# feiyeha/EGM-Unet

Measured on AMD Instinct MI355X. Metric: train images/sec at 3x512x512 bs=8/GPU, higher is better.
Workload: dtype bf16; 1 GPU; EGM-UNet GRFBUNet(3,2,base_c=32) fwd+5-term-loss+bwd+SGD, 8x3x512x512 per GPU (BASELINE.json configs[1]); global_batch=8, parallelism=dp1, launch=hipGraph replay, world_size=1

## Files before the change

### egm_unet_amd/csrc/conv_wgrad.hip

```cpp
#include "common.h"
#include "group.h"
#include <string.h>
#include <stdio.h>
#include <stdlib.h>
#include <type_traits>

typedef __attribute__((ext_vector_type(8))) __bf16 bf16x8_t;
typedef __attribute__((ext_vector_type(4))) short s16x4_t;
typedef __attribute__((ext_vector_type(8))) short s16x8_t;
typedef __attribute__((ext_vector_type(16))) float f32x16_t;
typedef __attribute__((ext_vector_type(4))) unsigned int u32x4_t;

int egm_conv_c7_wgrad_plan(int dtype, int N, int H, int W, int Cin, int Cout, int KH, int KW, int dil);
int egm_conv_c7_wgrad_launch(const void* x, int ldx, const void* dy, int lddy, float* slab, int nslab, int N, int H, int W, egm_stream_t s);
int egm_conv_c16d_wgrad_plan(int dtype, int N, int H, int W, int Cin, int Cout, int KH, int KW, int dil);
int egm_conv_c16d_wgrad_launch(const void* x, int ldx, const void* dy, int lddy, float* slab, int nslab, int N, int H, int W, int dil,
                               egm_stream_t s);

namespace {

constexpr int TH = 8, TW = 32;
constexpr int kMaxRowDil = 36;

template <typename T> struct WMma;
// ... 674 lines not shown
    if (sl == 0 && i < total) {
        s = (red[e] + red[64 + e]) + (red[128 + e] + red[192 + e]);
        const int ci = (int)(i % CinP), co = (int)((i / CinP) % CoutP), tap = (int)(i / ((long long)CinP * CoutP));
        if (co < CoutR && ci < CinR && (co / cout_g) == (ci / cin_g)) {
            const long long o = ((long long)co * cin_g + (ci % cin_g)) * taps + tap;
            dw[o] = accumulate ? dw[o] + s : s;
        }
    }
}


__global__ __launch_bounds__(1024) void wgrad_reduce_wide_kernel(const float* __restrict__ slab, float* __restrict__ dw, int nslab, int taps,
                                                                 int CoutP, int CinP, int CoutR, int CinR, int groups, int accumulate) {
    __shared__ float red[1024];
    const long long total = (long long)taps * CoutP * CinP;
    const int cin_g = CinR / groups, cout_g = CoutR / groups;
    const int e = threadIdx.x & 63, sl = threadIdx.x >> 6;
    const long long i = (long long)blockIdx.x * 64 + e;
    float s = 0.f;
    if (i < total)
        for (int k = sl; k < nslab; k += 16) s += slab[(long long)k * total + i];
    red[threadIdx.x] = s;
    __syncthreads();
    for (int w = 8; w > 0; w >>= 1) {
        if (sl < w) red[threadIdx.x] += red[threadIdx.x + w * 64];
        __syncthreads();
    }
    if (sl == 0 && i < total) {
        s = red[e];
        const int ci = (int)(i % CinP), co = (int)((i / CinP) % CoutP), tap = (int)(i / ((long long)CinP * CoutP));
        if (co < CoutR && ci < CinR && (co / cout_g) == (ci / cin_g)) {
            const long long o = ((long long)co * cin_g + (ci % cin_g)) * taps + tap;
            dw[o] = accumulate ? dw[o] + s : s;
        }
    }
}

struct WredEntry { const float* slab; float* dw; int nslab, taps, CoutP, CinP, CoutR, CinR, groups, accumulate, chunk0, pad; };
constexpr int kWredElems = 256;
__global__ __launch_bounds__(256) void wgrad_reduce_multi_kernel(const WredEntry* __restrict__ tab, int n) {
    __shared__ float4 red[256];
    const int s_t = egm_find_entry(tab, n, (long long)blockIdx.x);
    const int s_c = (int)((long long)blockIdx.x - (long long)tab[s_t].chunk0);
    const WredEntry w = tab[s_t];
    const long long total = (long long)w.taps * w.CoutP * w.CinP;
    const int cin_g = w.CinR / w.groups, cout_g = w.CoutR / w.groups;
    const int e = threadIdx.x & 63, sl = threadIdx.x >> 6;
    const long long i0 = (long long)s_c * kWredElems + e * 4;
    float4 s = make_float4(0.f, 0.f, 0.f, 0.f);
    if (i0 < total) {
        const float* src = w.slab + i0;
        int k = sl;
        for (; k + 4 < w.nslab; k += 8) {
            const float4 a = *reinterpret_cast<const float4*>(src + (long long)k * total);
            const float4 c = *reinterpret_cast<const float4*>(src + (long long)(k + 4) * total);
            s.x += a.x; s.y += a.y; s.z += a.z; s.w += a.w;
            s.x += c.x; s.y += c.y; s.z += c.z; s.w += c.w;
        }
        if (k < w.nslab) {
            const float4 a = *reinterpret_cast<const float4*>(src + (long long)k * total);
            s.x += a.x; s.y += a.y; s.z += a.z; s.w += a.w;
        }
    }
    red[threadIdx.x] = s;
    __syncthreads();
    if (sl == 0 && i0 < total) {
        const float4 r0 = red[e], r1 = red[64 + e], r2 = red[128 + e], r3 = red[192 + e];
        const float v[4] = {(r0.x + r1.x) + (r2.x + r3.x), (r0.y + r1.y) + (r2.y + r3.y), (r0.z + r1.z) + (r2.z + r3.z),
                            (r0.w + r1.w) + (r2.w + r3.w)};
#pragma unroll
        for (int j = 0; j < 4; ++j) {
            const long long i = i0 + j;
            const int ci = (int)(i % w.CinP), co = (int)((i / w.CinP) % w.CoutP), tap = (int)(i / ((long long)w.CinP * w.CoutP));
            if (co < w.CoutR && ci < w.CinR && (co / cout_g) == (ci / cin_g)) {
                const long long o = ((long long)co * cin_g + (ci % cin_g)) * w.taps + tap;
                w.dw[o] = w.accumulate ? w.dw[o] + v[j] : v[j];
            }
        }
    }
}

struct WgradPlan { int A, B, C, ntaps, ngroups, nsplit, nco_tiles, nci_tiles, npt, tiles_y, tiles_x, dma, ws, c7; size_t smem; long long slab_bytes; };

int wgrad_plan(int dtype, int N, int H, int W, int Cin, int Cout, int KH, int KW, int dil, WgradPlan* pl) {
    if (KH == 1 && KW == 1) dil = 1;
    pl->c7 = 0;
    {
        const int ns = egm_conv_c7_wgrad_plan(dtype, N, H, W, Cin, Cout, KH, KW, dil);
        if (ns > 0) {
            memset(pl, 0, sizeof(*pl));
            pl->c7 = 1; pl->ntaps = 7; pl->ngroups = 7; pl->nsplit = ns; pl->A = pl->B = 1; pl->C = 4;
            pl->slab_bytes = (long long)ns * KH * KW * Cout * Cin * (long long)sizeof(float);
            return EGM_OK;
        }
        const int nd = egm_conv_c16d_wgrad_plan(dtype, N, H, W, Cin, Cout, KH, KW, dil);
        if (nd > 0) {
            memset(pl, 0, sizeof(*pl));
            pl->c7 = 2; pl->ntaps = 3; pl->ngroups = 3; pl->nsplit = nd; pl->A = pl->B = 1; pl->C = 4;
            pl->slab_bytes = (long long)nd * KH * KW * Cout * Cin * (long long)sizeof(float);
            return EGM_OK;
        }
    }
    if (dil == 1) {
        if (KH == 3 && KW == 3) { pl->ntaps = 9; pl->ngroups = 1; }
        else if (KH == 1 && KW == 1) { pl->ntaps = 1; pl->ngroups = 1; }
        else if (KW == 5) { pl->ntaps = 5; pl->ngroups = KH; }
        else if (KW == 7) { pl->ntaps = 7; pl->ngroups = KH; }
        else return EGM_ERR_UNSUPPORTED;
    } else {
        const int rbp = dtype == EGM_BF16 ? 64 : 128;
        const int Ap = (dtype == EGM_F32 && Cout > 32 && Cin > 32) ? 1 : (Cout > 32 ? 2 : 1), Bp = Cin > 32 ? 2 : 1;
        const size_t row_smem = (size_t)Ap * TH * TW * rbp + (size_t)Bp * TH * (TW + 2 * dil) * rbp;
        if (KH == 3 && KW == 3 && dil <= kMaxRowDil && row_smem <= 156 * 1024 && W >= 128 && H >= 128 && Cin <= 32 && Cout <= 32) { pl->ntaps = 3; pl->ngroups = 3; }
        else { pl->ntaps = 1; pl->ngroups = KH * KW; }
    }
    int A = Cout > 32 ? 2 : 1, B = Cin > 32 ? 2 : 1;
    if (dtype == EGM_F32 && A * B == 4) A = 1;
    pl->A = A; pl->B = B; pl->C = 4 / (A * B);
    pl->nco_tiles = egm_cdiv(Cout, 32 * A); pl->nci_tiles = egm_cdiv(Cin, 32 * B);
    pl->tiles_y = egm_cdiv(H, TH); pl->tiles_x = egm_cdiv(W, TW); pl->npt = N * pl->tiles_y * pl->tiles_x;
    const int blocks_per_split = pl->nco_tiles * pl->nci_tiles * pl->ngroups;
    static const int per_cu_small = getenv("EGM_WGRAD_PER_CU") ? atoi(getenv("EGM_WGRAD_PER_CU")) : 2;
    static const int ws_on = getenv("EGM_WGRAD_WS") ? atoi(getenv("EGM_WGRAD_WS")) : 1;
    const bool ws_family = dtype == EGM_BF16 && ws_on && pl->ntaps >= 5;
    pl->ws = ws_family ? 1 : 0;
    int per_cu = ws_family ? 1 : ((pl->ntaps <= 3 && dtype == EGM_BF16) ? per_cu_small : 1);
    static const int ws_per_cu = getenv("EGM_WGRAD_WS_PER_CU") ? atoi(getenv("EGM_WGRAD_WS_PER_CU")) : 1;
    if (ws_family && ws_per_cu > 1 && A * B == 1 && pl->ntaps == 9) per_cu = ws_per_cu;
    int nsplit = 256 * per_cu / blocks_per_split;
    if (nsplit < 1) nsplit = 1;
    if (nsplit > pl->npt) nsplit = pl->npt;
    pl->nsplit = nsplit;
    const int rb = dtype == EGM_BF16 ? 64 : 128;
    const int wh = pl->ntaps == 9 ? 3 : 1, ww = pl->ntaps == 9 ? 3 : pl->ntaps;
    const int pw = (dil > 1 && pl->ntaps == 3) ? TW + 2 * dil : TW + ww - 1;
    pl->smem = (size_t)A * TH * TW * rb + (size_t)B * (TH + wh - 1) * pw * rb;
    static const int dma_off = getenv("EGM_WGRAD_NO_DMA") != nullptr;
    pl->dma = (dtype == EGM_BF16 && !pl->ws && !dma_off && A * B == 4 && pl->ntaps == 9 && 2 * pl->smem <= 156 * 1024) ? 1 : 0;
    if (pl->ws) pl->smem = (size_t)A * TH * TW * rb + (((size_t)B * (TH + wh - 1) * pw * rb + 4095) & ~(size_t)4095);
    if (pl->dma || pl->ws) pl->smem *= 2;
    const size_t red_bytes = pl->C > 1 ? (size_t)A * B * (pl->C - 1) * pl->ntaps * 16 * 64 * sizeof(float) : 0;
    if (pl->smem < red_bytes) pl->smem = red_bytes;
    pl->slab_bytes = (long long)nsplit * KH * KW * Cout * Cin * (long long)sizeof(float);
    return EGM_OK;
}

template <typename Single, typename Multi>
int launch_wgrad_group_impl(const EgmGroupRec* recs, int n, hipStream_t st, Single single, Multi multi, int threads, const char* what) {
    if (n == 1) {
        WgradParams first;
        memcpy(&first, recs[0].params, sizeof(WgradParams));
        const int* g3 = reinterpret_cast<const int*>(recs[0].params + sizeof(WgradParams));
        hipLaunchKernelGGL(single, dim3(g3[0], g3[1], g3[2]), dim3(threads), recs[0].smem, st, first);
        EGM_CHECK_LAUNCH(what);
        return EGM_OK;
    }
    WgradMulti m;
    size_t smem = 0;
    m.n = n; m.blk0[0] = 0;
    for (int i = 0; i < n; ++i) {
        memcpy(&m.p[i], recs[i].params, sizeof(WgradParams));
        const int* g3 = reinterpret_cast<const int*>(recs[i].params + sizeof(WgradParams));
        m.nx[i] = g3[0]; m.ny[i] = g3[1];
        m.blk0[i + 1] = m.blk0[i] + g3[0] * g3[1] * g3[2];
        if (recs[i].smem > smem) smem = recs[i].smem;
    }
    for (int i = n; i < EGM_GROUP_MAX; ++i) { m.p[i] = m.p[0]; m.nx[i] = m.ny[i] = 1; m.blk0[i + 1] = m.blk0[n]; }
    hipLaunchKernelGGL(multi, dim3(m.blk0[n]), dim3(threads), smem, st, m);
    EGM_CHECK_LAUNCH(what);
    return EGM_OK;
}
template <typename T, int NTAPS>
int launch_wgrad_group(const EgmGroupRec* recs, int n, hipStream_t st) {
    static bool attr_done = false;
    if (!attr_done) {
        hipError_t e = hipFuncSetAttribute(reinterpret_cast<const void*>(conv_wgrad_multi_kernel<T, NTAPS>),
                                           hipFuncAttributeMaxDynamicSharedMemorySize, 160 * 1024);
        if (e != hipSuccess) EGM_FAIL(EGM_ERR_LAUNCH, "conv_wgrad_multi: hipFuncSetAttribute: %s", hipGetErrorString(e));
        attr_done = true;
    }
    return launch_wgrad_group_impl(recs, n, st, conv_wgrad_kernel<T, NTAPS>, conv_wgrad_multi_kernel<T, NTAPS>, 256, "conv_wgrad (group)");
}
template <int NTAPS, int CC>
int launch_wgrad_ws_group(const EgmGroupRec* recs, int n, hipStream_t st) {
    static bool attr_done = false;
    if (!attr_done) {
        hipError_t e = hipFuncSetAttribute(reinterpret_cast<const void*>(conv_wgrad_ws_multi_kernel<NTAPS, CC>),
                                           hipFuncAttributeMaxDynamicSharedMemorySize, 160 * 1024);
        if (e != hipSuccess) EGM_FAIL(EGM_ERR_LAUNCH, "conv_wgrad_ws_multi: hipFuncSetAttribute: %s", hipGetErrorString(e));
        attr_done = true;
    }
    return launch_wgrad_group_impl(recs, n, st, conv_wgrad_ws_kernel<NTAPS, CC>, conv_wgrad_ws_multi_kernel<NTAPS, CC>, 512, "conv_wgrad_ws (group)");
}
inline bool wgrad_record(int (*fn)(const EgmGroupRec*, int, hipStream_t), const WgradParams& p, dim3 grid, size_t smem) {
    if (!egm_group_recording()) return false;
    static_assert(sizeof(WgradParams) + 3 * sizeof(int) <= sizeof(EgmGroupRec::params), "group record too small");
    EgmGroupRec r;
    r.launch = fn;
    memcpy(r.params, &p, sizeof(WgradParams));
    const int g3[3] = {(int)grid.x, (int)grid.y, (int)grid.z};
    memcpy(r.params + sizeof(WgradParams), g3, sizeof(g3));
    r.G = 0; r.grid = (int)(grid.x * grid.y * grid.z); r.smem = smem;
    egm_group_push(r);
    return true;
}
template <typename T, int NTAPS>
int launch_wgrad_4w(const WgradParams& p, const WgradPlan& pl, hipStream_t st) {
    static bool attr_done = false;
    if (!attr_done) {
        hipError_t e = hipFuncSetAttribute(reinterpret_cast<const void*>(conv_wgrad_kernel<T, NTAPS>),
                                           hipFuncAttributeMaxDynamicSharedMemorySize, 160 * 1024);
        if (e != hipSuccess) EGM_FAIL(EGM_ERR_LAUNCH, "conv_wgrad: hipFuncSetAttribute: %s", hipGetErrorString(e));
        attr_done = true;
    }
// ... 5 lines not shown
}
template <int NTAPS, int CC>
int launch_wgrad_ws_rot(const WgradParams& p, const WgradPlan& pl, hipStream_t st) {
    static bool attr_done = false;
    if (!attr_done) {
        hipError_t e = hipFuncSetAttribute(reinterpret_cast<const void*>(conv_wgrad_ws_kernel<NTAPS, CC>),
                                           hipFuncAttributeMaxDynamicSharedMemorySize, 160 * 1024);
        if (e != hipSuccess) EGM_FAIL(EGM_ERR_LAUNCH, "conv_wgrad_ws: hipFuncSetAttribute: %s", hipGetErrorString(e));
        attr_done = true;
    }
    dim3 grid(pl.nsplit, pl.nco_tiles * pl.nci_tiles, pl.ngroups);
    if (wgrad_record(&launch_wgrad_ws_group<NTAPS, CC>, p, grid, pl.smem)) return EGM_OK;
    hipLaunchKernelGGL((conv_wgrad_ws_kernel<NTAPS, CC>), grid, dim3(512), pl.smem, st, p);
    EGM_CHECK_LAUNCH("conv_wgrad_ws");
    return EGM_OK;
}
template <int NTAPS>
int launch_wgrad_ws(const WgradParams& p, const WgradPlan& pl, hipStream_t st) {
    if constexpr (NTAPS == 9) {
        static const bool rot_on = getenv("EGM_WGRAD_ROT") ? atoi(getenv("EGM_WGRAD_ROT")) != 0 : true;
        if (rot_on) {
            if (pl.C == 1) return launch_wgrad_ws_rot<NTAPS, 1>(p, pl, st);
            if (pl.C == 2) return launch_wgrad_ws_rot<NTAPS, 2>(p, pl, st);
            return launch_wgrad_ws_rot<NTAPS, 4>(p, pl, st);
        }
    }
    return launch_wgrad_ws_rot<NTAPS, 0>(p, pl, st);
}
template <typename T, int NTAPS>
int launch_wgrad(const WgradParams& p, const WgradPlan& pl, hipStream_t st) {
    if constexpr (sizeof(T) == 2 && NTAPS >= 5) {
        if (pl.ws) return launch_wgrad_ws<NTAPS>(p, pl, st);
    }
    return launch_wgrad_4w<T, NTAPS>(p, pl, st);
}

template <typename T>
int dispatch_wgrad(const WgradParams& p, const WgradPlan& pl, hipStream_t st) {
    switch (pl.ntaps) {
        case 9: return launch_wgrad<T, 9>(p, pl, st);
        case 7: return launch_wgrad<T, 7>(p, pl, st);
        case 5: return launch_wgrad<T, 5>(p, pl, st);
        case 3: return launch_wgrad<T, 3>(p, pl, st);
        case 1: return launch_wgrad<T, 1>(p, pl, st);
    }
    EGM_FAIL(EGM_ERR_UNSUPPORTED, "conv_wgrad: unsupported tap group %d", pl.ntaps);
}

}

extern "C" long long egm_conv_wgrad_workspace(int N, int H, int W, int Cin, int Cout, int KH, int KW) {
    WgradPlan pl;
    if (wgrad_plan(EGM_F32, N, H, W, Cin, Cout, KH, KW, 1, &pl) != EGM_OK) return -1;
    long long a = pl.slab_bytes;
    if (wgrad_plan(EGM_BF16, N, H, W, Cin, Cout, KH, KW, 1, &pl) != EGM_OK) return -1;
    if (pl.slab_bytes > a) a = pl.slab_bytes;
    if (wgrad_plan(EGM_BF16, N, H, W, Cin, Cout, KH, KW, 2, &pl) != EGM_OK) return -1;
    if (pl.slab_bytes > a) a = pl.slab_bytes;
    if (wgrad_plan(EGM_F32, N, H, W, Cin, Cout, KH, KW, 2, &pl) != EGM_OK) return -1;
    if (pl.slab_bytes > a) a = pl.slab_bytes;
    return a;
}

extern "C" int egm_conv_wgrad_kernel_name(int dtype, int N, int H, int W, int Cin, int Cout, int KH, int KW, int dil, char* buf, int buflen) {
    WgradPlan pl;
    if (KH == 1 && KW == 1) dil = 1;
    if (wgrad_plan(dtype, N, H, W, Cin, Cout, KH, KW, dil, &pl) != EGM_OK) return -1;
    char tmp[96];
    static const bool rot_on = getenv("EGM_WGRAD_ROT") ? atoi(getenv("EGM_WGRAD_ROT")) != 0 : true;
    if (pl.c7) snprintf(tmp, sizeof(tmp), pl.c7 == 1 ? "conv7x7_c16_wgrad_kernel" : "conv3x3d_c16_wgrad_kernel");
    else if (dtype == EGM_BF16 && pl.ws)
        snprintf(tmp, sizeof(tmp), "conv_wgrad_ws_kernel<%d, %d>", pl.ntaps, (pl.ntaps == 9 && rot_on) ? pl.C : 0);
    else
        snprintf(tmp, sizeof(tmp), "conv_wgrad_kernel<%s, %d>", dtype == EGM_BF16 ? "bf16_t" : "float", pl.ntaps);
    const int n = (int)strlen(tmp);
    if (buf != nullptr && buflen > 0) { strncpy(buf, tmp, (size_t)buflen - 1); buf[buflen - 1] = 0; }
    return n;
}
extern "C" int egm_conv_wgrad_slabs(int dtype, int N, int H, int W, int Cin, int Cout, int KH, int KW, int dil) {
    WgradPlan pl;
    if (KH == 1 && KW == 1) dil = 1;
    if (wgrad_plan(dtype, N, H, W, Cin, Cout, KH, KW, dil, &pl) != EGM_OK) return -1;
    return pl.nsplit;
}
extern "C" int egm_wgrad_reduce_chunk(void) { return kWredElems; }
extern "C" int egm_wgrad_reduce_multi(const void* table_dev, int n, long long total_chunks, egm_stream_t s) {
    EGM_REQUIRE(table_dev && n > 0 && total_chunks > 0 && total_chunks < (1LL << 30), "wgrad_reduce_multi: bad args");
    hipLaunchKernelGGL(wgrad_reduce_multi_kernel, dim3((unsigned)total_chunks), dim3(256), 0, (hipStream_t)s, (const WredEntry*)table_dev, n);
    EGM_CHECK_LAUNCH("wgrad_reduce_multi");
    return EGM_OK;
}

extern "C" int egm_conv_wgrad(int dtype, const void* x, int ldx, const void* dy, int lddy, float* dw, void* workspace, int N,
                              int H, int W, int Cin, int Cout, int CinR, int CoutR, int KH, int KW, int dil, int groups,
                              int accumulate, egm_stream_t s) {
    EGM_REQUIRE(x && dy && workspace, "conv_wgrad: null pointer");
    EGM_REQUIRE(N > 0 && H > 0 && W > 0, "conv_wgrad: bad shape");
    EGM_REQUIRE(Cin % 8 == 0 && Cout % 8 == 0 && Cin > 0 && Cout > 0, "conv_wgrad: padded channels must be multiples of 8");
    EGM_REQUIRE(CinR <= Cin && CoutR <= Cout && CinR > 0 && CoutR > 0 && groups > 0 && CinR % groups == 0 && CoutR % groups == 0,
                "conv_wgrad: bad real channel counts");
    EGM_REQUIRE(ldx >= Cin && lddy >= Cout && ldx % 8 == 0 && lddy % 8 == 0, "conv_wgrad: bad ld");
    EGM_REQUIRE(egm_aligned16(x) && egm_aligned16(dy) && egm_aligned16(workspace), "conv_wgrad: pointers must be 16-byte aligned");
    EGM_REQUIRE(dil >= 1 && (KH & 1) && (KW & 1), "conv_wgrad: bad kernel");
    if (KH == 1 && KW == 1) dil = 1;
    WgradPlan pl;
    if (wgrad_plan(dtype, N, H, W, Cin, Cout, KH, KW, dil, &pl) != EGM_OK)
        EGM_FAIL(EGM_ERR_UNSUPPORTED, "conv_wgrad: unsupported kernel %dx%d dil %d", KH, KW, dil);
    EGM_REQUIRE(pl.smem <= 160 * 1024, "conv_wgrad: LDS budget exceeded");
    WgradParams p;
    p.x = x; p.dy = dy; p.slab = (float*)workspace; p.ldx = ldx; p.lddy = lddy; p.N = N; p.H = H; p.W = W;
    p.Cin = Cin; p.Cout = Cout; p.KH = KH; p.KW = KW; p.dil = dil; p.tiles_y = pl.tiles_y; p.tiles_x = pl.tiles_x;
    p.npt = pl.npt; p.nsplit = pl.nsplit; p.A = pl.A; p.B = pl.B; p.C = pl.C; p.nci_tiles = pl.nci_tiles; p.ngroups = pl.ngroups;
    p.dma = pl.dma;
    hipStream_t st = (hipStream_t)s;
    int rc;
    const bool paused = dw != nullptr && egm_group_recording();
    if (paused) egm_group_set_recording(false);
    if (pl.c7 == 1) rc = egm_conv_c7_wgrad_launch(x, ldx, dy, lddy, (float*)workspace, pl.nsplit, N, H, W, s);
    else if (pl.c7 == 2) rc = egm_conv_c16d_wgrad_launch(x, ldx, dy, lddy, (float*)workspace, pl.nsplit, N, H, W, dil, s);
    else if (dtype == EGM_BF16) rc = dispatch_wgrad<bf16_t>(p, pl, st);
    else if (dtype == EGM_F32) rc = dispatch_wgrad<float>(p, pl, st);
    else rc = EGM_ERR_ARG;
    if (paused) egm_group_set_recording(true);
    if (rc == EGM_ERR_ARG && dtype != EGM_BF16 && dtype != EGM_F32) EGM_FAIL(EGM_ERR_ARG, "conv_wgrad: unknown dtype %d", dtype);
    if (rc != EGM_OK) return rc;
    if (dw == nullptr) return EGM_OK;
    return egm_wgrad_reduce((const float*)workspace, dw, pl.nsplit, KH * KW, Cout, Cin, CoutR, CinR, groups, accumulate, s);
}

extern "C" int egm_conv_wgrad_multi(int dtype, const egm_conv_wgrad_desc* d, int n, egm_stream_t s) {
    EGM_REQUIRE(d && n > 0 && n <= EGM_WGRAD_MULTI_MAX, "conv_wgrad_multi: 1..%d convolutions per call", EGM_WGRAD_MULTI_MAX);
    EGM_REQUIRE(!egm_group_recording(), "conv_wgrad_multi: called inside an open launch group");
    int rc = egm_group_begin();
    if (rc != EGM_OK) return rc;
    for (int i = 0; i < n && rc == EGM_OK; ++i)
        rc = egm_conv_wgrad(dtype, d[i].x, d[i].ldx, d[i].dy, d[i].lddy, nullptr, d[i].slabs, d[i].N, d[i].H, d[i].W, d[i].Cin, d[i].Cout, d[i].Cin_real,
                            d[i].Cout_real, d[i].KH, d[i].KW, d[i].dil, d[i].groups, 0, s);
    if (rc != EGM_OK) { egm_group_abort(); return rc; }
    return egm_group_end(s);
}

extern "C" int egm_wgrad_reduce(const float* slabs, float* dw, int nslab, int taps, int CoutP, int CinP, int CoutR, int CinR, int groups,
                                int accumulate, egm_stream_t s) {
    EGM_REQUIRE(slabs && dw && nslab > 0 && taps > 0 && CoutP > 0 && CinP > 0 && CoutR > 0 && CoutR <= CoutP && CinR > 0 && CinR <= CinP && groups > 0,
                "wgrad_reduce: bad args");
    hipStream_t st = (hipStream_t)s;
    const long long total = (long long)taps * CoutP * CinP;
    const int grid = (int)((total + 63) / 64);
    if (nslab >= 256 && grid < 1024)
        hipLaunchKernelGGL(wgrad_reduce_wide_kernel, dim3(grid), dim3(1024), 0, st, slabs, dw, nslab, taps, CoutP, CinP, CoutR, CinR, groups, accumulate);
    else
        hipLaunchKernelGGL(wgrad_reduce_kernel, dim3(grid), dim3(256), 0, st, slabs, dw, nslab, taps, CoutP, CinP, CoutR, CinR, groups, accumulate);
    EGM_CHECK_LAUNCH("wgrad_reduce");
    return EGM_OK;
}
```

### egm_unet_amd/ops.py

```python
import ctypes
import os
import struct
import threading
import weakref
from collections import namedtuple

import torch
from torch.autograd import Function, Variable

from ._lib import ACT_NONE, ACT_RELU, ACT_SIGMOID, dtype_code, lib, ptr, stream


def pad8(c: int) -> int:
    return (c + 7) // 8 * 8


def _nhwc(t: torch.Tensor):
    assert t.dim() == 4, t.shape
    N, H, W, C = t.shape
    s = t.stride()
    ok = (s[3] == 1 and s[2] % 8 == 0 and s[2] >= C and s[1] == W * s[2] and s[0] == H * W * s[2]
          and t.data_ptr() % 16 == 0 and C % 8 == 0)
    if not ok:
        if C % 8:
            raise RuntimeError(f"egm_unet_amd: channel count {C} is not a multiple of 8")
        t = t.contiguous()
        s = t.stride()
    return t, s[2]


def _npix(t):
    return t.shape[0] * t.shape[1] * t.shape[2]


def _f32(n, device, zero=False):
    return (torch.zeros if zero else torch.empty)(n, dtype=torch.float32, device=device)


class _Switch:

    def __init__(self, env, default, doc=None, parse=lambda v: v != "0"):
        self.on, self.__doc__ = parse(os.environ.get(env, default)), doc

    def __call__(self, enabled=None):
        if enabled is not None:
            self.on = type(self.on)(enabled)
        return type(self.on)(self.on)


_zero_pools = {}


def _zero_grad_vec(n, device):
    pool = _zero_pools.get(device)
    if pool is None or pool[0].numel() < pool[1] + n:
        if torch.cuda.is_current_stream_capturing():
            return torch.zeros(n, dtype=torch.float32, device=device)
        pool = _zero_pools[device] = [torch.zeros(max(1 << 16, 4 * n), dtype=torch.float32, device=device), 0]
    off = pool[1]
    pool[1] = off + n
    return pool[0][off:off + n]


def _bn_conv_bias_grad(Cout, dy, training, device):
    return _zero_grad_vec(Cout, device) if training else _channel_sum(dy)[0, :Cout]


def _slot_or_new(out_slot, shape, dtype, device):
    if out_slot is None:
        t = torch.empty(shape, dtype=dtype, device=device)
        return t, shape[3]
    t = out_slot[0]
    v, ld = _nhwc(t)
    if v.data_ptr() != t.data_ptr() or tuple(t.shape) != tuple(shape) or t.dtype != dtype:
        raise RuntimeError(f"egm_unet_amd: output slot {tuple(t.shape)}/{t.dtype} does not fit result {tuple(shape)}/{dtype}")
    return t, ld


def cat_slots(N, H, W, channels, dtype, device):
    buf = torch.empty((N, H, W, sum(channels)), dtype=dtype, device=device)
    views, off = [], 0
    for c in channels:
        views.append(buf[..., off:off + c])
# ... 164 lines not shown
        st = model._egm_prepack = {"dtype": dtype, "convs": convs, "bufs": bufs, "table": DeviceTable(), "stamp": None}
    convs, bufs = st["convs"], st["bufs"]
    if not convs:
        return
    stamp = (_weight_generation[0], tuple(m.weight._version for m in convs), tuple(m.weight.data_ptr() for m in convs))
    if stamp == st["stamp"]:
        return
    L = lib()
    chunk = L.cdll.egm_conv_pack_chunk()
    blob, chunks = bytearray(), 0
    for m, (wf, wd) in zip(convs, bufs):
        Cout, Cin_g, KH, KW = m.weight.shape
        Cin = Cin_g * m.groups
        blob += struct.pack("<QQQiiiiiiii", m.weight.data_ptr(), wf.data_ptr(), wd.data_ptr(), Cout, Cin, pad8(Cout), pad8(Cin), KH, KW,
                            m.groups, chunks)
        chunks += (KH * KW * pad8(Cout) * pad8(Cin) + chunk - 1) // chunk
    dev = convs[0].weight.device
    table = st["table"].get(bytes(blob), dev)
    L.call("egm_conv_pack_multi", dtype_code(dtype), ptr(table), len(convs), chunks, stream())
    for m, (wf, wd) in zip(convs, bufs):
        w = m.weight
        key = (w.data_ptr(), w._version, _weight_generation[0], dtype, m.groups, tuple(w.shape))
        _pack_cache[id(w)] = (key, wf, wd, weakref.ref(w))
    st["stamp"] = stamp


_conv_uses = {}


def _note_conv_use(weight):
    ent = _conv_uses.get(id(weight))
    if ent is None or ent[0]() is not weight or ent[1] != _weight_generation[0]:
        ent = _conv_uses[id(weight)] = [weakref.ref(weight), _weight_generation[0], 0, 0]
        if len(_conv_uses) > 4096:
            for k in [k for k, v in _conv_uses.items() if v[0]() is None]:
                del _conv_uses[k]
    ent[2] += 1
    ent[3] = max(ent[3], ent[2])


def _sole_conv_use(weight):
    ent = _conv_uses.get(id(weight))
    if ent is None or ent[0]() is not weight:
        return False
    sole = ent[3] == 1
    ent[2] -= 1
    if ent[2] <= 0:
        del _conv_uses[id(weight)]
    return sole


_DEFER_WGRAD = os.environ.get("EGM_DEFER_WGRAD", "1") != "0"
merge_wgrads = _Switch("EGM_MERGE_WGRAD", "1",
                       """Get / set whether the slab kernels of deferred weight gradients are launched together when backward ends (merged
                       launches).""")
defer_bgrads = _Switch("EGM_DEFER_BGRAD", "1",
                       """Get / set whether conv bias gradients are left to the one multi-tensor pass at the end of backward.""")
fuse_dz = _Switch("EGM_FUSE_DZ", "1",
                  """Get / set whether BatchNorm backward computes dz on the fly from the classifier / MCALayer behind it (tests compare both
                  ways).""")


def _wgrad_deferrable(weight):
    return (_DEFER_WGRAD and _sole_conv_use(weight) and weight.is_leaf and weight.grad is None
            and not weight._backward_hooks and not torch.is_grad_enabled())


_wgrad_table, _wgrad_table_partial, _bgrad_table, _bgrad_table_partial = DeviceTable(), DeviceTable(), DeviceTable(), DeviceTable()
_BSUM_ENTRY = struct.Struct("<3Qq6i")
_WGRAD_DESC = struct.Struct("<3Q14i")
_wgrad_names = {}


def _wgrad_kernel_of(dt, N, H, W, CinP, CoutP, KH, KW, dil):
    key = (dt, N, H, W, CinP, CoutP, KH, KW, dil)
    name = _wgrad_names.get(key)
    if name is None:
        buf = ctypes.create_string_buffer(96)
        lib().cdll.egm_conv_wgrad_kernel_name(dt, N, H, W, CinP, CoutP, KH, KW, dil, ctypes.cast(buf, ctypes.c_void_p), 96)
        name = _wgrad_names[key] = buf.value
    return name


_Slab = namedtuple("_Slab", "dt x ldx gy ldg ws N H W CinP CoutP Cin Cout KH KW dil groups")
_Wgrad = namedtuple("_Wgrad", "ws param nslab taps CoutP CinP Cout Cin groups gref gptr")
_Bgrad = namedtuple("_Bgrad", "gy ldg npix C Cout param gref gptr")


def _handed_over(queue, ready_only, name):
    todo, later = [], []
    for ent in queue:
        grad = ent.param.grad
        if ent.gref() is not None or (grad is not None and grad.data_ptr() == ent.gptr):
            todo.append(ent)
        elif ready_only:
            later.append(ent)
        elif grad is not None:
            raise RuntimeError(f"deferred conv {name} gradient lost its destination: {name}.grad exists but is not the buffer backward() "
                               f"returned (tensor hook / gradient copy); set EGM_DEFER_{name[0].upper()}GRAD=0 for this model")
    queue[:] = later
    return todo


_runs = {}


class _BackwardRun:
    __slots__ = ("id", "slabs", "wgrads", "bgrads", "dz", "__weakref__")

    def __init__(self, run_id):
        self.id, self.slabs, self.wgrads, self.bgrads, self.dz = run_id, [], [], [], {}

    def finish(self):
        _runs.pop(self.id, None)
        if self.dz:
            kinds = [v[1][0] for v in self.dz.values()]
            self.dz.clear()
            raise RuntimeError(f"egm_unet_amd: deferred BatchNorm gradients {kinds} were never consumed (the tensor between the producer and "
                               "its BatchNorm had another consumer); call ops.fuse_dz(False)")
        self.flush()

    def flush(self, ready_only=False):
        self.flush_bgrads(ready_only)
        self.launch_slabs()
        self.reduce_wgrads(ready_only)

    def flush_bgrads(self, ready_only=False):
        todo = _handed_over(self.bgrads, ready_only, "bias") if self.bgrads else None
        if not todo:
            return
        L = lib()
        by_dtype = {}
        for e in todo:
            by_dtype.setdefault(e.gy.dtype, []).append(e)
        for dtype, ents in by_dtype.items():
            dev = ents[0].gy.device
            nblks = [L.query("egm_channel_partials_blocks", e.npix, e.C) for e in ents]
            ws = torch.empty(sum(nb * 2 * e.C for nb, e in zip(nblks, ents)), dtype=torch.float32, device=dev)
            blob1, blob2, b1, b2, off = bytearray(), bytearray(), 0, 0, 0
            for nb, e in zip(nblks, ents):
                part = ws.data_ptr() + 4 * off
                blob1 += _BSUM_ENTRY.pack(e.gy.data_ptr(), part, e.gptr, e.npix, e.ldg, e.C, e.Cout, nb, b1, 0)
                blob2 += _BSUM_ENTRY.pack(e.gy.data_ptr(), part, e.gptr, e.npix, e.ldg, e.C, e.Cout, nb, b2, 0)
                b1 += nb; b2 += e.C // 8; off += nb * 2 * e.C
            _bgrad_table.reserve(dev); _bgrad_table_partial.reserve(dev)
            table = (_bgrad_table_partial if ready_only else _bgrad_table).get(bytes(blob1 + blob2), dev)
            L.call("egm_bias_grad_multi", dtype_code(dtype), ptr(table), len(ents), b1, b2, stream())

    def launch_slabs(self):
        if not self.slabs:
            return
        L, st = lib(), stream()
        todo, self.slabs = self.slabs, []
        buckets = {}
        for e in todo:
            buckets.setdefault((e.dt, _wgrad_kernel_of(e.dt, e.N, e.H, e.W, e.CinP, e.CoutP, e.KH, e.KW, e.dil)), []).append(e)
        per = 4
        for (dt, _name), ents in buckets.items():
            for i in range(0, len(ents), per):
                blob = b"".join(_WGRAD_DESC.pack(e.x.data_ptr(), e.gy.data_ptr(), e.ws.data_ptr(), e.ldx, e.ldg, e.N, e.H, e.W, e.CinP, e.CoutP,
                                                 e.Cin, e.Cout, e.KH, e.KW, e.dil, e.groups, 0) for e in ents[i:i + per])
                L.call("egm_conv_wgrad_multi", dt, blob, len(ents[i:i + per]), st)

    def reduce_wgrads(self, ready_only=False):
        todo = _handed_over(self.wgrads, ready_only, "weight") if self.wgrads else None
        if not todo:
            return
        blob, chunks = bytearray(), 0
        per = lib().cdll.egm_wgrad_reduce_chunk()
        for e in todo:
            blob += struct.pack("<QQiiiiiiiiii", e.ws.data_ptr(), e.gptr, e.nslab, e.taps, e.CoutP, e.CinP, e.Cout, e.Cin, e.groups, 0, chunks, 0)
            chunks += (e.taps * e.CoutP * e.CinP + per - 1) // per
        dev = todo[0].param.device
        _wgrad_table.reserve(dev); _wgrad_table_partial.reserve(dev)
        table = (_wgrad_table_partial if ready_only else _wgrad_table).get(bytes(blob), dev)
        lib().call("egm_wgrad_reduce_multi", ptr(table), len(todo), chunks, stream())


def _run(create=True):
    run_id = torch._C._current_graph_task_id()
    ref = _runs.get(run_id)
    run = None if ref is None else ref()
    if run is None and create:
        run = _BackwardRun(run_id)
        _runs[run_id] = weakref.ref(run, lambda _ref: _runs.pop(run_id, None))
        Variable._execution_engine.queue_callback(run.finish)
    return run


def flush_ready_wgrads():
    run = _run(create=False)
    if run is not None:
        run.flush(ready_only=True)


def _queue_wgrad(ws, weight, nslab, taps, CoutP, CinP, Cout, Cin, groups, gw):
    _run().wgrads.append(_Wgrad(ws, weight, nslab, taps, CoutP, CinP, Cout, Cin, groups, weakref.ref(gw), gw.data_ptr()))


def _defer_dz(standin, payload):
    _run().dz[standin.data_ptr()] = (standin, payload)


def _take_dz(g):
    run = _run(create=False)
    return run.dz.pop(g.data_ptr(), None) if run is not None and run.dz else None


def _bias_grad(gy, Cout, bias=None, defer=False):
    if (defer and defer_bgrads.on and bias is not None and bias.is_leaf and bias.grad is None and not bias._backward_hooks
            and not torch.is_grad_enabled()):
        gy, ldg = _nhwc(gy)
        gb = torch.empty(Cout, dtype=torch.float32, device=gy.device)
        _run().bgrads.append(_Bgrad(gy, ldg, _npix(gy), gy.shape[3], Cout, bias, weakref.ref(gb), gb.data_ptr()))
        return gb
    return _channel_sum(gy)[0, :Cout]


def _channel_sum(t):
    t, ld = _nhwc(t)
    C, npix = t.shape[3], _npix(t)
    nb = lib().query("egm_channel_partials_blocks", npix, C)
    part = _f32(nb * 2 * C, t.device)
    out = _f32((2, C), t.device)
    lib().call("egm_channel_sums", dtype_code(t.dtype), ptr(t), ld, npix, C, ptr(part), stream())
    lib().call("egm_reduce_tiles", ptr(part), nb, C, ptr(out), stream())
    return out


class Lazy:
    __slots__ = ("y", "coef", "act")

    def __init__(self, y, coef, act):
        self.y, self.coef, self.act = y, coef, act

    shape = property(lambda self: self.y.shape)
    dtype = property(lambda self: self.y.dtype)
    device = property(lambda self: self.y.device)

    def materialize(self, out=None):
        return _Materialize.apply(self.y, self.coef, self.act, None if out is None else [out])


def materialize(x, out=None):
    if isinstance(x, Lazy):
# ... 1951 lines not shown
```

### include/egm_hip.h

```cpp
#ifndef EGM_HIP_H
#define EGM_HIP_H

#ifdef __cplusplus
extern "C" {
#endif

typedef void* egm_stream_t;

enum egm_status { EGM_OK = 0, EGM_ERR_ARG = -1, EGM_ERR_LAUNCH = -2, EGM_ERR_UNSUPPORTED = -3 };
enum egm_dtype { EGM_F32 = 0, EGM_BF16 = 1 };
enum egm_act { EGM_ACT_NONE = 0, EGM_ACT_RELU = 1, EGM_ACT_SIGMOID = 2, EGM_ACT_SILU = 3  };

int egm_version(void);
const char* egm_last_error(void);
int egm_device_ok(void);

int egm_nchw_to_nhwc(int dtype, const void* src_f32, void* dst, int ld, int N, int C, int H, int W, egm_stream_t s);
int egm_nhwc_to_nchw(int dtype, const void* src, int ld, void* dst_f32, int N, int C, int H, int W, egm_stream_t s);

int egm_conv_pack(int dtype, const void* w_oihw_f32, void* wf, void* wd, int Cout, int Cin, int KH, int KW, int groups,
                  egm_stream_t s);
int egm_conv_pack_chunk(void);
int egm_conv_pack_multi(int dtype, const void* table_dev, int n, long long total_chunks, egm_stream_t s);
int egm_group_begin(void);
int egm_group_end(egm_stream_t s);
int egm_group_abort(void);
int egm_conv_tile_mode(int mode);
int egm_conv_tile_debug(int dbg);
int egm_conv_c7_mode(int mode);
int egm_conv_split_ok(int dtype, int N, int H, int W, int Cin, int Cout, int KH, int KW, int dil, int csplit);
int egm_conv_fwd_split(int dtype, const void* x, int ldx, const void* wf, void* y, int ldy, void* y2, int ldy2, int csplit, int N,
                       int H, int W, int Cin, int Cout, int KH, int KW, int dil, egm_stream_t s);
int egm_conv_kernel_name(int dtype, int N, int H, int W, int Cin, int Cout, int KH, int KW, int dil, char* buf, int buflen);
int egm_conv_fwd(int dtype, const void* x, int ldx, const void* wf, const void* bias_f32, int bias_n, void* y, int ldy,
                 float* stats, int N, int H, int W, int Cin, int Cout, int KH, int KW, int dil, egm_stream_t s);
int egm_conv_stats_tiles(int dtype, int N, int H, int W, int Cin, int Cout, int KH, int KW, int dil);
int egm_conv_fwd_act(int dtype, const void* x, int ldx, const void* wf, const void* bias_f32, int bias_n, void* y, int ldy, int N, int H,
                     int W, int Cin, int Cout, int KH, int KW, int dil, int act, egm_stream_t s);
int egm_conv_fold_chunk(void);
int egm_conv_fold_pack_multi(int dtype, const void* table_dev, int n, long long total_chunks, egm_stream_t s);
int egm_argmax_u8(const float* logits, const unsigned char* lut, unsigned char* out, int N, int C, int H, int W, egm_stream_t s);
long long egm_conv_wgrad_workspace(int N, int H, int W, int Cin, int Cout, int KH, int KW);
int egm_conv_wgrad(int dtype, const void* x, int ldx, const void* dy, int lddy, float* dw_oihw_f32, void* workspace,
                   int N, int H, int W, int Cin, int Cout, int CinR, int CoutR, int KH, int KW, int dil, int groups,
                   int accumulate, egm_stream_t s);
int egm_conv_wgrad_kernel_name(int dtype, int N, int H, int W, int Cin, int Cout, int KH, int KW, int dil, char* buf, int buflen);
#define EGM_WGRAD_MULTI_MAX 4
typedef struct egm_conv_wgrad_desc {
    const void* x; const void* dy; void* slabs;
    int ldx, lddy, N, H, W, Cin, Cout, Cin_real, Cout_real, KH, KW, dil, groups, pad_;
} egm_conv_wgrad_desc;
int egm_conv_wgrad_multi(int dtype, const egm_conv_wgrad_desc* descs, int n, egm_stream_t stream);
int egm_conv_wgrad_slabs(int dtype, int N, int H, int W, int Cin, int Cout, int KH, int KW, int dil);
int egm_wgrad_reduce(const float* slabs, float* dw_oihw_f32, int nslab, int taps, int CoutP, int CinP, int CoutR, int CinR, int groups,
                     int accumulate, egm_stream_t s);
int egm_wgrad_reduce_chunk(void);
int egm_wgrad_reduce_multi(const void* table_dev, int n, long long total_chunks, egm_stream_t s);
int egm_dwconv3_fwd(int dtype, const void* x, int ldx, const float* w, const float* b, const float* scale, void* y, int ldy,
                    int N, int H, int W, int C, egm_stream_t s);
long long egm_dwconv3_bwd_workspace(int N, int H, int W, int C);
int egm_dwconv3_bwd(int dtype, const void* x, int ldx, const void* dy, int lddy, const float* w, const float* b,
                    const float* scale, void* dx, int lddx, float* dw, float* db, float* dscale, void* workspace,
                    int N, int H, int W, int C, egm_stream_t s);

int egm_channel_partials_blocks(long long npix, int C);
int egm_channel_sums(int dtype, const void* x, int ld, long long npix, int C, float* partials, egm_stream_t s);
int egm_reduce_tiles(const float* tiles, int ntiles, int C, float* out_2xC, egm_stream_t s);
int egm_reduce_tiles_batched(const float* tiles, int batch, int ntiles, int C, float* out, egm_stream_t s);
typedef struct { const void* x; float* part; float* out; long long npix; int ld, C, Cout, nblk, chunk0, pad; } egm_bsum_entry;
int egm_bias_grad_multi(int dtype, const void* table_dev, int n, long long blocks1, long long blocks2, egm_stream_t s);

int egm_bn_finalize(const float* stats, int ntiles, long long count, const float* gamma, const float* beta, float eps,
                    float momentum, float* running_mean, float* running_var, float* scale, float* shift,
                    float* save_mean, float* save_rstd, int C, int C_real, egm_stream_t s);
int egm_bn_eval_coeffs(const float* gamma, const float* beta, const float* running_mean, const float* running_var,
                       float eps, float* scale, float* shift, float* save_mean, float* save_rstd, int C, int C_real,
                       egm_stream_t s);
int egm_bn_act_fwd(int dtype, const void* y, int ldy, const float* scale, const float* shift, int act, void* z, int ldz,
                   long long npix, int C, egm_stream_t s);
int egm_bn_act_bwd_reduce(int dtype, const void* dz, int lddz, const void* y, int ldy, const float* scale,
                          const float* shift, const float* save_mean, const float* save_rstd, int act, float* partials,
                          long long npix, int C, egm_stream_t s);
int egm_bn_act_bwd_apply(int dtype, const void* dz, int lddz, const void* y, int ldy, const float* scale,
                         const float* shift, const float* save_mean, const float* save_rstd, int act, int train,
                         const float* sums, void* dy, int lddy, long long npix, int C, egm_stream_t s);
int egm_bn_act_cls_fwd(int dtype, const void* y, int ldy, const float* scale, const float* shift, int act, void* z, int ldz,
                       const float* w_cls, int nc, int ldw, const float* bias, float* logits_nchw, int N, int H, int W, int C,
                       egm_stream_t s);
int egm_bn_cls_bwd_reduce(int dtype, const void* dlogits, int lddl, const float* w_cls, int nc, int ldw, const void* y, int ldy,
                          const float* scale, const float* shift, const float* save_mean, const float* save_rstd, int act,
                          float* partials, long long npix, int C, egm_stream_t s);
int egm_bn_cls_bwd_apply(int dtype, const void* dlogits, int lddl, const float* w_cls, int nc, int ldw, const void* y, int ldy,
                         const float* scale, const float* shift, const float* save_mean, const float* save_rstd, int act, int train,
                         const float* sums, void* dy, int lddy, long long npix, int C, egm_stream_t s);
int egm_bn_mca_bwd_reduce(int dtype, const void* dxo, int ldd, const float* gates, const float* coef, int no_spatial, const void* y,
                          int ldy, const float* scale, const float* shift, const float* save_mean, const float* save_rstd, int act,
                          float* partials, int N, int H, int W, int C, egm_stream_t s);
int egm_bn_mca_bwd_apply(int dtype, const void* dxo, int ldd, const float* gates, const float* coef, int no_spatial, const void* y,
                         int ldy, const float* scale, const float* shift, const float* save_mean, const float* save_rstd, int act,
                         int train, const float* sums, void* dy, int lddy, int N, int H, int W, int C, egm_stream_t s);
int egm_bn_bwd_coefs(const float* partials, int ntiles, long long count, const float* scale, const float* shift,
                     const float* save_mean, const float* save_rstd, int train, float* sums_2xC, float* cf_4xC, int C,
                     egm_stream_t s);

#define EGM_BN_MULTI_MAX 4
enum egm_bn_multi_pass { EGM_BN_MULTI_FINALIZE = 0, EGM_BN_MULTI_FWD = 1, EGM_BN_MULTI_BWD_REDUCE = 2, EGM_BN_MULTI_BWD_COEFS = 3,
                         EGM_BN_MULTI_BWD_APPLY = 4 };
typedef struct egm_bn_desc {
    const void* y;  void* z;  const void* dz;  void* dy;
    float* coef;
    const float* stats;
    const float* gamma;  const float* beta;  float* running_mean;  float* running_var;
    float* partials;  float* sums;  float* cf4;
    long long npix;
    int ldy, ldz, lddz, lddy, ntiles, nblocks, C, C_real, act, train;
    float eps, momentum;
} egm_bn_desc;
int egm_bn_multi(int dtype, int pass, const egm_bn_desc* descs, int n, egm_stream_t s);

enum egm_ew_mode { EGM_EW_GATE = 0, EGM_EW_SAR = 1 };
int egm_bn_ew_fwd(int dtype, int mode, const void* y, int ldy, const float* scale, const float* shift, int act, const void* p,
                  int ldp, float alpha, void* out, int ldo, long long npix, int C, egm_stream_t s);
int egm_bn_ew_bwd_reduce(int dtype, int mode, const void* g, int ldg, const void* q, int ldq, const void* y, int ldy,
                         const float* scale, const float* shift, const float* save_mean, const float* save_rstd, int act,
                         float alpha, float* partials, long long npix, int C, egm_stream_t s);
int egm_bn_ew_bwd_apply(int dtype, int mode, const void* g, int ldg, const void* q, int ldq, const void* y, int ldy,
                        const float* cf_4xC, int act, float alpha, void* dy, int lddy, void* dp, int lddp, long long npix, int C,
                        egm_stream_t s);

typedef struct egm_pw_head {
    const void* x;  const void* w;  const void* wd;
    const float* bias;  const float* gamma;  const float* beta;  float* running_mean;  float* running_var;
    float* coef;
    const void* p;  void* out;
    const void* g;  const void* q;  void* dp;
    float* sums;  float* cf4;  float* dw;  float* dbias;
// ... 276 lines not shown
```

Baseline: 673.1 images/s.

## Cap wgrad split-K slabs for large 3x3 convs and balance multi-launch grouping

For large ws-family 3x3 weight-gradient convs with a 2x2 tile config, large slab footprint and many pixel tiles, the split count is capped so each block walks at least a minimum number of tiles. This shrinks the fp32 slab traffic and the reduction cost. On the Python side, wgrad descriptors within a kernel bucket are regrouped by a small exhaustive search. It estimates per-CU wave steps from block counts and walk lengths so the multi-launches are better balanced. The risk is lower parallelism per launch and search overhead, though results are cached and replayed under a graph.

```diff
diff --git a/egm_unet_amd/csrc/conv_wgrad.hip b/egm_unet_amd/csrc/conv_wgrad.hip
--- a/egm_unet_amd/csrc/conv_wgrad.hip
+++ b/egm_unet_amd/csrc/conv_wgrad.hip
@@ -780,7 +780,10 @@
 
 struct WgradPlan { int A, B, C, ntaps, ngroups, nsplit, nco_tiles, nci_tiles, npt, tiles_y, tiles_x, dma, ws, c7; size_t smem; long long slab_bytes; };
 
-int wgrad_plan(int dtype, int N, int H, int W, int Cin, int Cout, int KH, int KW, int dil, WgradPlan* pl) {
+constexpr int kWgradMinTiles = 32, kWgradRuleTiles = 8;
+constexpr long long kWgradRuleBytes = 32LL << 20;
+
+int wgrad_plan(int dtype, int N, int H, int W, int Cin, int Cout, int KH, int KW, int dil, WgradPlan* pl, int min_tiles = -1) {
     if (KH == 1 && KW == 1) dil = 1;
     pl->c7 = 0;
     {
@@ -828,6 +831,14 @@
     int nsplit = 256 * per_cu / blocks_per_split;
     if (nsplit < 1) nsplit = 1;
     if (nsplit > pl->npt) nsplit = pl->npt;
+    static const int min_tiles_env = getenv("EGM_WGRAD_MIN_TILES") ? atoi(getenv("EGM_WGRAD_MIN_TILES")) : kWgradMinTiles;
+    const int T = min_tiles < 0 ? min_tiles_env : min_tiles;
+    if (T > 0 && ws_family && pl->ntaps == 9 && A * B == 4 && (long long)nsplit * KH * KW * Cout * Cin * (long long)sizeof(float) >= kWgradRuleBytes &&
+        pl->npt >= kWgradRuleTiles * nsplit) {
+        int few = pl->npt / T;
+        if (few < 1) few = 1;
+        if (few < nsplit) nsplit = few;
+    }
     pl->nsplit = nsplit;
     const int rb = dtype == EGM_BF16 ? 64 : 128;
     const int wh = pl->ntaps == 9 ? 3 : 1, ww = pl->ntaps == 9 ? 3 : pl->ntaps;
@@ -999,6 +1010,25 @@
     if (KH == 1 && KW == 1) dil = 1;
     if (wgrad_plan(dtype, N, H, W, Cin, Cout, KH, KW, dil, &pl) != EGM_OK) return -1;
     return pl.nsplit;
+}
+extern "C" int egm_conv_wgrad_slabs_at(int dtype, int N, int H, int W, int Cin, int Cout, int KH, int KW, int dil, int min_tiles) {
+    WgradPlan pl;
+    if (KH == 1 && KW == 1) dil = 1;
+    if (min_tiles < 0 || wgrad_plan(dtype, N, H, W, Cin, Cout, KH, KW, dil, &pl, min_tiles) != EGM_OK) return -1;
+    return pl.nsplit;
+}
+extern "C" int egm_conv_wgrad_blocks(int dtype, int N, int H, int W, int Cin, int Cout, int KH, int KW, int dil) {
+    WgradPlan pl;
+    if (KH == 1 && KW == 1) dil = 1;
+    if (wgrad_plan(dtype, N, H, W, Cin, Cout, KH, KW, dil, &pl) != EGM_OK) return -1;
+    if (pl.c7) return pl.nsplit;
+    return pl.nsplit * pl.nco_tiles * pl.nci_tiles * pl.ngroups;
+}
+extern "C" int egm_conv_wgrad_walk(int dtype, int N, int H, int W, int Cin, int Cout, int KH, int KW, int dil) {
+    WgradPlan pl;
+    if (KH == 1 && KW == 1) dil = 1;
+    if (wgrad_plan(dtype, N, H, W, Cin, Cout, KH, KW, dil, &pl) != EGM_OK) return -1;
+    return pl.c7 ? 1 : egm_cdiv(pl.npt, pl.nsplit);
 }
 extern "C" int egm_wgrad_reduce_chunk(void) { return kWredElems; }
 extern "C" int egm_wgrad_reduce_multi(const void* table_dev, int n, long long total_chunks, egm_stream_t s) {
diff --git a/egm_unet_amd/ops.py b/egm_unet_amd/ops.py
--- a/egm_unet_amd/ops.py
+++ b/egm_unet_amd/ops.py
@@ -1,4 +1,5 @@
 import ctypes
+import itertools
 import os
 import struct
 import threading
@@ -329,6 +330,56 @@
     return name
 
 
+_wgrad_shapes = {}
+_wgrad_groupings = {}
+_CUS = 256
+
+
+def _wgrad_shape_of(e):
+    key = (e.dt, e.N, e.H, e.W, e.CinP, e.CoutP, e.KH, e.KW, e.dil)
+    v = _wgrad_shapes.get(key)
+    if v is None:
+        v = _wgrad_shapes[key] = (lib().query("egm_conv_wgrad_blocks", *key), lib().query("egm_conv_wgrad_walk", *key))
+    return v
+
+
+def _launch_steps(members):
+    steps = -(-sum(b * w for b, w in members) // _CUS)
+    for w in {w for _, w in members}:
+        steps = max(steps, w * -(-sum(b for b, w2 in members if w2 >= w) // _CUS))
+    return steps
+
+
+def _even_launches(ents, per, shape_of=_wgrad_shape_of):
+    queue_order = [ents[i:i + per] for i in range(0, len(ents), per)]
+    n = len(queue_order)
+    if n <= 1 or n > 3:
+        return queue_order
+    shapes = tuple(shape_of(e) for e in ents)
+    best = _wgrad_groupings.get((shapes, per))
+    if best is None:
+        cost_of = lambda groups: sum(_launch_steps([shapes[i] for i in g]) for g in groups)
+        best, best_cost = None, cost_of([range(i, min(i + per, len(ents))) for i in range(0, len(ents), per)])
+
+        def search(rest, groups, cost):
+            nonlocal best, best_cost
+            if cost >= best_cost or len(groups) + -(-len(rest) // per) > n:
+                return
+            if not rest:
+                best, best_cost = [list(g) for g in groups], cost
+                return
+            first, others = rest[0], rest[1:]
+            for k in range(min(per - 1, len(others)), -1, -1):
+                for mates in itertools.combinations(others, k):
+                    g = (first,) + mates
+                    search([i for i in others if i not in mates], groups + [g], cost + _launch_steps([shapes[i] for i in g]))
+        search(list(range(len(ents))), [], 0)
+        best = _wgrad_groupings[(shapes, per)] = best or False
+    if not best:
+        return queue_order
+    return [[ents[i] for i in sorted(g, key=lambda i: (-shapes[i][1], i))] for g in best]
+
+
 _Slab = namedtuple("_Slab", "dt x ldx gy ldg ws N H W CinP CoutP Cin Cout KH KW dil groups")
 _Wgrad = namedtuple("_Wgrad", "ws param nslab taps CoutP CinP Cout Cin groups gref gptr")
 _Bgrad = namedtuple("_Bgrad", "gy ldg npix C Cout param gref gptr")
@@ -404,10 +455,10 @@
             buckets.setdefault((e.dt, _wgrad_kernel_of(e.dt, e.N, e.H, e.W, e.CinP, e.CoutP, e.KH, e.KW, e.dil)), []).append(e)
         per = 4
         for (dt, _name), ents in buckets.items():
-            for i in range(0, len(ents), per):
+            for group in _even_launches(ents, per):
                 blob = b"".join(_WGRAD_DESC.pack(e.x.data_ptr(), e.gy.data_ptr(), e.ws.data_ptr(), e.ldx, e.ldg, e.N, e.H, e.W, e.CinP, e.CoutP,
-                                                 e.Cin, e.Cout, e.KH, e.KW, e.dil, e.groups, 0) for e in ents[i:i + per])
-                L.call("egm_conv_wgrad_multi", dt, blob, len(ents[i:i + per]), st)
+                                                 e.Cin, e.Cout, e.KH, e.KW, e.dil, e.groups, 0) for e in group)
+                L.call("egm_conv_wgrad_multi", dt, blob, len(group), st)
 
     def reduce_wgrads(self, ready_only=False):
         todo = _handed_over(self.wgrads, ready_only, "weight") if self.wgrads else None
diff --git a/include/egm_hip.h b/include/egm_hip.h
--- a/include/egm_hip.h
+++ b/include/egm_hip.h
@@ -52,6 +52,9 @@
 } egm_conv_wgrad_desc;
 int egm_conv_wgrad_multi(int dtype, const egm_conv_wgrad_desc* descs, int n, egm_stream_t stream);
 int egm_conv_wgrad_slabs(int dtype, int N, int H, int W, int Cin, int Cout, int KH, int KW, int dil);
+int egm_conv_wgrad_slabs_at(int dtype, int N, int H, int W, int Cin, int Cout, int KH, int KW, int dil, int min_tiles);
+int egm_conv_wgrad_blocks(int dtype, int N, int H, int W, int Cin, int Cout, int KH, int KW, int dil);
+int egm_conv_wgrad_walk(int dtype, int N, int H, int W, int Cin, int Cout, int KH, int KW, int dil);
 int egm_wgrad_reduce(const float* slabs, float* dw_oihw_f32, int nslab, int taps, int CoutP, int CinP, int CoutR, int CinR, int groups,
                      int accumulate, egm_stream_t s);
 int egm_wgrad_reduce_chunk(void);
```

Result: no change. 679.5 images/s (median of 6 runs) (+1.0%).
